# p-mc-grath/DMMFODS

Measured on AMD Instinct MI355X. Metric: training images/sec at 1280x1920 RGB+LiDAR, higher is better.
Workload: dtype f16; 1 GPU; C2 d121 early-fusion 6ch b4 1280x1920; key=c2, per_gpu_batch=4, global_batch=4, height=1280, width=1920, storage_dtype=fp16, accumulate=fp32, parallelism=dp1, weights=random-init (reference init, seed 123)

## Files before the change

dmmfods_amd/csrc/bw1.hip:

```cpp
#include <algorithm>
#include <cstdio>
#include <cstdlib>
#include <type_traits>

#include "common.h"
#include "dispatch.h"
#include "gather.h"
#include "isa.h"
#include "pointwise.h"

namespace dmm {

#ifndef B1_DBG
#define B1_DBG 0
#endif
#ifndef B1_LATE_PREFETCH
#define B1_LATE_PREFETCH 0
#endif
#ifndef B1_RAW_BAR
#define B1_RAW_BAR 0
#endif
#ifndef B1_NT
#define B1_NT 0
#endif
// ... 264 lines not shown
      }
    };
    if (cvalid) { if (UNC && full) finish(std::true_type()); else finish(std::false_type()); }
    fold_to_lds<16, SLOT, B1_CT>(s1, s2, red, cs, cvalid, lane);
    }
#if B1_RAW_BAR
    lds_barrier();
#else
    __syncthreads();
#endif
  }

  if (tid < B1_CT && c0 + tid < a.N) {
    const size_t rep = (size_t)(blockIdx.x & (STAT_REPS - 1)) * a.stat_stride;
    const double S1 = red[fold_slot<16, SLOT>(0, tid)];
    double S2 = red[fold_slot<16, SLOT>(1, tid)];
    if constexpr (UNC) S2 = (S2 - (double)kc[2 * B1_CT + tid] * S1) * (double)kc[3 * B1_CT + tid];
    atomic_add_f64(a.red1 + rep + c0 + tid, S1);
    atomic_add_f64(a.red2 + rep + c0 + tid, S2);
  }
  const int c = c0 + 32 * wave + r;
  if constexpr (PART) {
    float* slot = g.part + ((size_t)split * g.nct + ct) * B1_SLOT_FLOATS + (size_t)wave * (B1_NB * 32);
#pragma unroll
    for (int j = 0; j < 4; ++j)
#pragma unroll
      for (int i = 0; i < 16; ++i) {
        const int n = 32 * j + (i & 3) + 8 * (i >> 2) + 4 * h;
        slot[n * 32 + r] = accw[j][i];
      }
  } else if (!(B1_DBG & 1) && c < g.wC) {
    const size_t chunk = (size_t)(c0 / 32 + wave);
#pragma unroll
    for (int j = 0; j < 4; ++j)
#pragma unroll
      for (int i = 0; i < 16; ++i) {
        const int n = 32 * j + (i & 3) + 8 * (i >> 2) + 4 * h;
        atomic_add_f32(g.dpack + (chunk * g.dNpad + n) * 32 + r, accw[j][i]);
      }
  }
  if (B1_DBG & 1) {
    float s = 0.f;
#pragma unroll
    for (int j = 0; j < 4; ++j)
#pragma unroll
      for (int i = 0; i < 16; ++i) s += accw[j][i];
    if (s == 1.2345e33f) g.dpack[0] = s;
  }
}

template <typename T, int PQ, bool ACC, bool PART>
static hipError_t launch_bw1_t(const Bw1Args& g, int nwg, hipStream_t st) {
  return launch_lds<bw1_kernel<T, PQ, ACC, PART>>(B1_LDS, nwg, NTHREADS, B1_LDS, st, g);
}

bool bw1_eligible(const WgradArgs& w, const ConvArgs& d, int dtype, unsigned deny) {
  if (((deny >> IMPL_BW1) & 1u) || dtype == DT_F32 || w.nseg != 1 || d.nseg != 1 || d.pool2) return false;
  const Seg& wx = w.seg[0];
  const Seg& wg = w.dy;
  const Seg& dg = d.seg[0];
  if (wx.mode != G_PLAIN || wx.istride != 1 || wx.ntaps != 1 || wx.taps[0] != 0 || wx.scale == nullptr || wx.C % 32) return false;
  if (wg.mode != G_PLAIN || wg.istride != 1 || wg.ntaps != 1 || wg.taps[0] != 0 || wg.scale != nullptr || wg.C != B1_NB) return false;
  if (dg.mode != G_PLAIN || dg.istride != 1 || dg.ntaps != 1 || dg.taps[0] != 0 || dg.scale != nullptr || dg.C != B1_NB || dg.Cpad != B1_NB) return false;
  if (dg.src != wg.src || dg.ld != wg.ld || dg.q != wg.q || dg.src2 != wg.src2) return false;
  if (w.N != B1_NB || w.Npad != B1_NB || w.M != d.M || d.N != wx.C || d.Npad % 32) return false;
  if (d.bx != wx.src || d.ldbx != wx.ld || d.bscale != wx.scale || d.bshift != wx.shift) return false;
  if (d.out == nullptr || d.ostride != 1 || d.Hout != d.Ho || d.Wout != d.Wo || wx.Hs != d.Ho || wx.Ws != d.Wo) return false;
  const double span = 2.0 * (double)d.M;
  if (span * d.ldbx >= 4294967296.0 || span * d.ldo >= 4294967296.0 || span * dg.ld >= 4294967296.0 || span * dg.ld2 >= 4294967296.0) return false;
  return true;
}

Bw1Geom bw1_geometry(const ConvArgs& a) {
  Bw1Geom q;
  q.nct = (a.N + B1_CT - 1) / B1_CT;
  q.ntiles = (a.M + B1_TM - 1) / B1_TM;
  constexpr int cus = DESIGN_CUS;
  static const int per_cu = lab_int("DMM_BW1_PER_CU", 2);
  int nsplit = std::max(1, (per_cu * cus + q.nct - 1) / q.nct);
  nsplit = std::min(nsplit, std::max(1, q.ntiles / 4));
  q.tiles_per_wg = (q.ntiles + nsplit - 1) / nsplit;
  q.nsplit = (q.ntiles + q.tiles_per_wg - 1) / q.tiles_per_wg;
  q.xcd_group = (q.nct > 1 && q.nsplit >= 32 && q.tiles_per_wg >= 8) ? 1 : 0;
  q.nwg = q.xcd_group ? ((q.nsplit + 7) / 8) * 8 * q.nct : q.nsplit * q.nct;
  return q;
}

static bool g_bw1_part = !lab_flag("DMM_NO_BW1_PART");

static bool bw1_uses_part(const Bw1Args& g, const Bw1Geom& q) {
  return g_bw1_part && g.part != nullptr && q.nsplit * q.nct <= g.part_slots && q.nsplit > 1;
}

hipError_t launch_bw1(const Bw1Args& g0, int dtype, hipStream_t st) {
  Bw1Args g = g0;
  const ConvArgs& a = g.c;
  if (a.M <= 0) return hipSuccess;
  const Bw1Geom q = bw1_geometry(a);
  note_impl(IMPL_BW1);
  g.nct = q.nct; g.ntiles = q.ntiles; g.tiles_per_wg = q.tiles_per_wg; g.xcd_group = q.xcd_group; g.nsplit = q.nsplit;
  const int nwg = q.nwg;
  const int pq = a.seg[0].q ? 2 : 0;
  const bool acc = a.accumulate != 0;
  const bool part = bw1_uses_part(g, q);
#define B1_GO(T) \
  (part ? (pq ? (acc ? launch_bw1_t<T, 2, true, true>(g, nwg, st) : launch_bw1_t<T, 2, false, true>(g, nwg, st))     \
              : (acc ? launch_bw1_t<T, 0, true, true>(g, nwg, st) : launch_bw1_t<T, 0, false, true>(g, nwg, st)))    \
        : (pq ? (acc ? launch_bw1_t<T, 2, true, false>(g, nwg, st) : launch_bw1_t<T, 2, false, false>(g, nwg, st))   \
              : (acc ? launch_bw1_t<T, 0, true, false>(g, nwg, st) : launch_bw1_t<T, 0, false, false>(g, nwg, st))))
  if (dtype == DT_F16) return B1_GO(f16);
  return B1_GO(bf16);
#undef B1_GO
}

__global__ __launch_bounds__(256) void bw1_reduce_kernel(const float* __restrict__ part, float* __restrict__ dpack, int nct, int nsplit, int nfloats) {
  const int e = (blockIdx.x * 256 + threadIdx.x) * 4;
  if (e >= nct * B1_SLOT_FLOATS) return;
  f32x4 s = {0.f, 0.f, 0.f, 0.f};
  const float* p = part + e;
  const size_t pitch = (size_t)nct * B1_SLOT_FLOATS;
  int k = 0;
  for (; k + 16 <= nsplit; k += 16) {
    f32x4 v[16];
#pragma unroll
    for (int u = 0; u < 16; ++u) v[u] = __builtin_nontemporal_load((const f32x4*)(p + (size_t)(k + u) * pitch));
#pragma unroll
    for (int u = 0; u < 16; u += 4) s += (v[u] + v[u + 1]) + (v[u + 2] + v[u + 3]);
  }
  for (; k + 4 <= nsplit; k += 4) {
    const f32x4 v0 = *(const f32x4*)(p + (size_t)k * pitch), v1 = *(const f32x4*)(p + (size_t)(k + 1) * pitch);
    const f32x4 v2 = *(const f32x4*)(p + (size_t)(k + 2) * pitch), v3 = *(const f32x4*)(p + (size_t)(k + 3) * pitch);
    s += (v0 + v1) + (v2 + v3);
  }
  for (; k < nsplit; ++k) s += *(const f32x4*)(p + (size_t)k * pitch);
  if (e < nfloats) *(f32x4*)(dpack + e) = s;
}

hipError_t launch_bw1_reduce(const Bw1Args& g, hipStream_t st) {
  const ConvArgs& a = g.c;
  if (a.M <= 0) return hipSuccess;
  const Bw1Geom q = bw1_geometry(a);
  if (!bw1_uses_part(g, q)) return hipSuccess;
  const int nfloats = ((g.wC + 31) / 32) * g.dNpad * 32;
  const int nthreads = q.nct * B1_SLOT_FLOATS / 4;
  hipLaunchKernelGGL(bw1_reduce_kernel, dim3((nthreads + 255) / 256), dim3(256), 0, st, g.part, g.dpack, q.nct, q.nsplit, nfloats);
  return hipGetLastError();
}

}
```

dmmfods_amd/csrc/conv3.hip:

```cpp
#include <algorithm>
#include <cstdio>
#include <cstdlib>
#include <type_traits>

#include "common.h"
#include "dispatch.h"
#include "gather.h"
#include "isa.h"

namespace dmm {

constexpr int C3_TH = 8, C3_TW = 16;
#ifndef C3_DBG
#define C3_DBG 0
#endif
constexpr int C3_WRING = 3;
#ifndef C3_RAW_EPI_BAR
#define C3_RAW_EPI_BAR 0
#endif

struct Conv3Args {
  ConvArgs c;
  int tiles_y, tiles_x, ntiles;
  int dymin0, dxmin0;
// ... 271 lines not shown
      for (int gc = 0; gc < GC; ++gc) {
        const int ck = grp * GC + gc;
        if (ck < NCH) {
#pragma unroll
          for (int s = 0; s < 2; ++s) {
            V av = z;
            if constexpr (SEG0) {
              if (ck < NCH0) av = *(const V*)(halo + abase + toffs[ck / (SEG0 ? CG : 1)] + (ck % (SEG0 ? CG : 1)) * 64 + s * 32);
            }
            if constexpr (SEG1) if (ck >= NCH0) {
              const int o = off1[2 * (ck - NCH0) + s];
              const V ld = *(const V*)(halo1 + (o >= 0 ? o : 0));
              av = o >= 0 ? ld : z;
            }
#pragma unroll
            for (int t = 0; t < NT; ++t) {
              const V bv = *(const V*)(Bp + (gc * BN + 32 * t + r) * 64 + (((2 * s + h) ^ bsw) << 4));
              acc[t] = mma16(av, bv, acc[t]);
            }
          }
        }
      }
    }
    if (grp + 2 < NGRP) vm_lds_barrier<NPW>();
    else vm_lds_barrier<0>();
  }
  constexpr bool PERSIST = EPI == EPI_STORE;
  const int lnext = lt + gridDim.x;
  const bool more = PERSIST && lnext < nitems;
  if (more) { decode(lnext); load_halo(); }
  if (!((C3_DBG & 8) && acc[0][0] != 123.f)) {
  T* Cs = (T*)smem;
  constexpr int CPITCH = BN + 8;
  float ps1[NT], ps2[NT];
#pragma unroll
  for (int t = 0; t < NT; ++t) {
    ps1[t] = 0.f; ps2[t] = 0.f;
#pragma unroll
    for (int i = 0; i < 16; ++i) {
      const int row = 32 * wave + (i & 3) + 8 * (i >> 2) + 4 * h;
      const T v = from_f32<T>(acc[t][i]);
      Cs[row * CPITCH + 32 * t + r] = v;
      if (EPI == EPI_STORE && rowpix[row] >= 0) { const float f = to_f32(v); ps1[t] += f; ps2[t] = fmaf(f, f, ps2[t]); }
    }
  }
  if constexpr (EPI == EPI_STORE) {
#pragma unroll
    for (int t = 0; t < NT; ++t) {
      wpart[(wave * 2 + h) * BN + 32 * t + r] = fold_swap32(ps1[t], ps2[t]);
    }
  }
  if constexpr (PERSIST && C3_RAW_EPI_BAR) lds_barrier();
  else __syncthreads();

  if constexpr (EPI == EPI_STORE) {
    T* out = (T*)a.out;
#pragma unroll
    for (int i = 0; i < NIT; ++i) {
      const int row = rr + RPP * i;
      const int pix = rowpix[row];
      if (pix < 0 || !colvalid) continue;
      *(V*)(out + (size_t)pix * a.ldo + n) = *(const V*)(Cs + row * CPITCH + cv * SLOT);
    }
    if (!(a.stat_sum == nullptr || (C3_DBG & 32)))
    if (!(C3_DBG & 16) && tid < 2 * BN) {
      const int col = tid % BN, which = tid / BN;
      if (col < a.N) {
        double s = 0.0;
#pragma unroll
        for (int w = 0; w < 4; ++w) s += (double)wpart[(w * 2 + which) * BN + col];
        red[tid] += s;
      }
    }
  } else {
    float s1[SLOT], s2[SLOT];
#pragma unroll
    for (int i = 0; i < SLOT; ++i) { s1[i] = 0.f; s2[i] = 0.f; }
    T* gout = (T*)a.out;
    float sc[SLOT], sh[SLOT], mu[SLOT], is[SLOT];
    if (colvalid) {
      load_f32s<SLOT>(a.bscale + n, sc); load_f32s<SLOT>(a.bshift + n, sh);
      load_f32s<SLOT>(a.bmean + n, mu); load_f32s<SLOT>(a.binvstd + n, is);
    }
    constexpr bool TWO_PASS = !SEG0 && SEG1;
    const bool fin = TWO_PASS && a.eq != nullptr;
    float qv[TWO_PASS ? SLOT : 1], rv[TWO_PASS ? SLOT : 1];
    if constexpr (TWO_PASS) {
#pragma unroll
      for (int e = 0; e < SLOT; ++e) { qv[e] = 0.f; rv[e] = 0.f; }
      if (fin && colvalid) { load_f32s<SLOT>(a.eq + n, qv); load_f32s<SLOT>(a.er + n, rv); }
    }
#pragma unroll
    for (int i = 0; i < NIT; ++i) {
      if (ppre[i] < 0) continue;
      const int row = rr + RPP * i;
      float av[SLOT], xf[SLOT], gf[SLOT];
      vec_to_f32<T>(*(const V*)(Cs + row * CPITCH + cv * SLOT), av);
      vec_to_f32<T>(xpre[i], xf);
      if (a.accumulate && gout != nullptr) vec_to_f32<T>(*(const V*)(gout + (size_t)ppre[i] * a.ldo + n), gf);
#pragma unroll
      for (int e = 0; e < SLOT; ++e) {
        const float dz = (fmaf(xf[e], sc[e], sh[e]) > 0.f) ? av[e] : 0.f;
        s1[e] += dz;
        s2[e] = fmaf(dz, (xf[e] - mu[e]) * is[e], s2[e]);
        gf[e] = ((a.accumulate && gout != nullptr) ? gf[e] : 0.f) + sc[e] * dz;
        if constexpr (TWO_PASS) gf[e] += fmaf(rv[e], xf[e], qv[e]);
      }
      if (gout != nullptr) *(V*)(gout + (size_t)ppre[i] * a.ldo + n) = f32_to_vec<T>(gf);
    }
    if (a.red1 != nullptr) {
      fold_to_lds<NCV, SLOT, BN>(s1, s2, red, cv, colvalid, lane);
      __syncthreads();
      if (!(C3_DBG & (16 | 32)) && tid < BN && tid < a.N) {
        const size_t rep = (size_t)(blockIdx.x & (STAT_REPS - 1)) * a.stat_stride;
        atomic_add_f64(a.red1 + rep + tid, red[fold_slot<NCV, SLOT>(0, tid)]);
        atomic_add_f64(a.red2 + rep + tid, red[fold_slot<NCV, SLOT>(1, tid)]);
      }
    }
  }
  }
  if (!more) break;
  lt = lnext;
  if constexpr (PERSIST && C3_RAW_EPI_BAR) lds_barrier();
  else __syncthreads();
  }
  if constexpr (EPI == EPI_STORE) {
    if (!(a.stat_sum == nullptr || (C3_DBG & (16 | 32))) && tid < 2 * BN) {
      const int col = tid % BN, which = tid / BN;
      if (col < a.N) {
        const size_t rep = (size_t)(blockIdx.x & (STAT_REPS - 1)) * a.stat_stride;
        atomic_add_f64((which ? a.stat_sq : a.stat_sum) + rep + col, red[tid]);
      }
    }
  }
}

typedef hipError_t (*C3Inst)(const Conv3Args& g, hipStream_t st);

template <typename T, int CS, int SPAN, int TSPAN, int TSTR, int NT, int GC, int EPI, int PRO>
static hipError_t launch_c3(const Conv3Args& g, hipStream_t st) {
  typedef Conv3Cfg<T, CS, SPAN, TSPAN, TSTR, NT, GC> SM;
  static_assert(SM::bytes <= 80 * 1024, "two workgroups per CU");
  constexpr auto kern = conv3_kernel<T, CS, SPAN, TSPAN, TSTR, NT, GC, EPI, PRO>;
  const hipError_t e = lds_limit<kern>(SM::bytes > 48 * 1024 ? SM::bytes : 0);
  if (e != hipSuccess) return e;
  static const int cus = device_cus();
  static const int rounds = lab_int("DMM_C3_ROUNDS", 1);
  const int per_cu = std::min(4, (160 * 1024) / SM::bytes);
  int nwg = g.ntiles * (g.c.nphase > 0 ? g.c.nphase : 1);
  if (EPI == EPI_STORE && rounds > 0 && nwg > per_cu * cus * rounds) nwg = per_cu * cus * rounds / 8 * 8;
  return launch_lds<kern>(0, nwg, NTHREADS, SM::bytes, st, g);
}

template <typename T>
static C3Inst c3_instance(int epi, int pro, int cs, int span, int tspan, int tstr, int nt) {
  if (epi == EPI_STORE && pro == 1) {
    if (tspan < 0 && span == 2 && nt == 1 && cs == 16) return launch_c3<T, 16, 2, -1, 1, 1, 4, EPI_STORE, 1>;
    if (tspan < 0 && span == 2 && nt == 1 && cs == 8) return launch_c3<T, 8, 2, -1, 1, 1, 2, EPI_STORE, 1>;
    if (tspan == 2 && tstr == 2 && span == 1 && nt == 2 && cs == 16) return launch_c3<T, 16, 1, 2, 2, 2, 2, EPI_STORE, 1>;
  }
  if (epi == EPI_BNBWD && tspan < 0 && span == 2) {
    if (cs == 4 && nt == 4 && pro == 2) return launch_c3<T, 4, 2, -1, 1, 4, 1, EPI_BNBWD, 2>;
    if (cs == 4 && nt == 4 && pro == 0) return launch_c3<T, 4, 2, -1, 1, 4, 1, EPI_BNBWD, 0>;
    if (cs == 4 && nt == 2 && pro == 2) return launch_c3<T, 4, 2, -1, 1, 2, 1, EPI_BNBWD, 2>;
    if (cs == 4 && nt == 2 && pro == 0) return launch_c3<T, 4, 2, -1, 1, 2, 1, EPI_BNBWD, 0>;
    if (cs == 8 && nt == 1 && pro == 0) return launch_c3<T, 8, 2, -1, 1, 1, 2, EPI_BNBWD, 0>;
    if (cs == 8 && nt == 1 && pro == 2) return launch_c3<T, 8, 2, -1, 1, 1, 2, EPI_BNBWD, 2>;
  }
  if (epi == EPI_STORE && cs == 0 && tspan == 6 && tstr == 2 && pro == 0 && nt == 2) return launch_c3<T, 0, 0, 6, 2, 2, 2, EPI_STORE, 0>;
  if (epi == EPI_BNBWD && cs == 0 && tspan == 4 && tstr == 1 && pro == 0) {
    if (nt == 2) return launch_c3<T, 0, 0, 4, 1, 2, 2, EPI_BNBWD, 0>;
    if (nt == 1) return launch_c3<T, 0, 0, 4, 1, 1, 2, EPI_BNBWD, 0>;
  }
  return nullptr;
}

static bool tap_box(const Seg& sg, int& dymin, int& dxmin, int& span) {
  int dymax = -128, dxmax = -128;
  dymin = 127; dxmin = 127;
  for (int t = 0; t < sg.ntaps; ++t) {
    const int dy = (int)(signed char)(sg.taps[t] & 0xff), dx = (int)(signed char)((sg.taps[t] >> 8) & 0xff);
    dymin = dy < dymin ? dy : dymin; dymax = dy > dymax ? dy : dymax;
    dxmin = dx < dxmin ? dx : dxmin; dxmax = dx > dxmax ? dx : dxmax;
  }
  span = dymax - dymin;
  if (span < 0 || span > 6 || dxmax - dxmin != span || sg.ntaps != (span + 1) * (span + 1)) return false;
  bool seen[49] = {false};
  for (int t = 0; t < sg.ntaps; ++t) {
    const int dy = (int)(signed char)(sg.taps[t] & 0xff) - dymin, dx = (int)(signed char)((sg.taps[t] >> 8) & 0xff) - dxmin;
    if (seen[dy * (span + 1) + dx]) return false;
    seen[dy * (span + 1) + dx] = true;
  }
  return true;
}

struct Conv3Launch {
  Conv3Args g;
  C3Inst run;
  int shape[8];
};

bool conv3_resolve(const ConvArgs& a, int dtype, int epi, Resolved& r) {
  if (dtype == DT_F32 || a.nseg < 1 || a.nseg > 2 || a.pool2 || (epi != EPI_STORE && epi != EPI_BNBWD)) return false;
  const Seg& sg = a.seg[0];
  if (a.Npad % 32 || a.Npad > 128) return false;
  Conv3Launch& l = r.put<Conv3Launch>();
  Conv3Args& g = l.g;
  g.c = a;
  g.dymin0 = g.dxmin0 = g.dymin1 = g.dxmin1 = 0;
  int cs = 0, span = 0, tspan = -1, tstr = 1;
  auto thin_ok = [&](const Seg& s1, int stride) {
    return s1.mode == G_PLAIN && s1.istride == stride && s1.C == 8 && s1.Cpad == 8 && s1.Hs == stride * a.Ho && s1.Ws == stride * a.Wo &&
           s1.q == nullptr && tap_box(s1, g.dymin1, g.dxmin1, tspan);
  };
  if (a.nseg == 1 && sg.C == 8 && sg.istride == 2) {
    tstr = 2;
    if (epi != EPI_STORE || !thin_ok(sg, 2) || tspan != 6 || sg.scale != nullptr) return false;
  } else if (a.nseg == 1 && sg.C == 8) {
    if (!thin_ok(sg, 1) || tspan != 4 || sg.scale != nullptr) return false;
  } else {
    if (sg.mode != G_PLAIN || sg.istride != 1 || sg.C % 32 || sg.Cpad != sg.C || sg.Hs != a.Ho || sg.Ws != a.Wo) return false;
    if (!tap_box(sg, g.dymin0, g.dxmin0, span) || span < 1 || span > 2) return false;
    cs = sg.C / 8;
    if (a.nseg == 2) {
      tstr = 2;
      if (!thin_ok(a.seg[1], 2) || tspan != 2 || (a.seg[1].scale != nullptr) != (sg.scale != nullptr)) return false;
    }
  }
  if (a.nphase < 0 || a.nphase > 4) return false;
  if (a.nphase > 0) {
    if (epi != EPI_STORE || a.nseg != 2 || sg.ntaps != 4 || a.seg[1].ntaps != 9) return false;
    for (int ph = 0; ph < a.nphase; ++ph) {
      Seg t0 = sg, t1 = a.seg[1];
      for (int t = 0; t < 4; ++t) t0.taps[t] = a.ph_taps0[ph][t];
      for (int t = 0; t < 9; ++t) t1.taps[t] = a.ph_taps1[ph][t];
      int y0, x0, y1, x1, sp0, sp1;
      if (!tap_box(t0, y0, x0, sp0) || sp0 != span || !tap_box(t1, y1, x1, sp1) || sp1 != tspan || a.ph_wpack[ph] == nullptr ||
          a.ph_py[ph] < 0 || a.ph_py[ph] >= a.ostride || a.ph_px[ph] < 0 || a.ph_px[ph] >= a.ostride)
        return false;
      g.ph_dymin0[ph] = (signed char)y0; g.ph_dxmin0[ph] = (signed char)x0; g.ph_dymin1[ph] = (signed char)y1; g.ph_dxmin1[ph] = (signed char)x1;
    }
  }
  if (a.nseg == 1 && (a.ostride != 1 || a.Hout != a.Ho || a.Wout != a.Wo)) return false;
  if (cs == 0 && tspan == 6 && a.Npad != 64) return false;
  const int pro = sg.scale ? 1 : (sg.q ? 2 : 0);
  if (epi == EPI_BNBWD && a.accumulate && a.out == nullptr) return false;
  if ((a.eq != nullptr) != (a.er != nullptr)) return false;
  if (a.eq != nullptr && !(epi == EPI_BNBWD && cs == 0 && tspan == 4 && tstr == 1 && pro == 0 && a.out != nullptr && !a.accumulate &&
                           a.red1 == nullptr && a.red2 == nullptr))
    return false;
  g.tiles_y = (a.Ho + C3_TH - 1) / C3_TH;
  g.tiles_x = (a.Wo + C3_TW - 1) / C3_TW;
  g.ntiles = a.B * g.tiles_y * g.tiles_x;
  const int nt = a.Npad / 32;
  const int shape[8] = {epi, pro, cs, span, tspan, tstr, nt, a.M};
// ... 16 lines not shown
```

dmmfods_amd/csrc/pointwise.hip:

```cpp
#include <type_traits>

#include "common.h"
#include "gather.h"
#include "pointwise.h"

namespace dmm {

thread_local int g_last_impl = IMPL_AUTO;
thread_local unsigned g_impl_mask = 0;

template <typename T>
__global__ __launch_bounds__(256) void convert_input_kernel(ConvertArgs a) {
  __shared__ double red[16];
  if (threadIdx.x < 16) red[threadIdx.x] = 0.0;
  __syncthreads();
  const size_t plane = (size_t)a.H * a.W;
  const size_t npix = (size_t)a.B * plane;
  double s1[8], s2[8];
#pragma unroll
  for (int c = 0; c < 8; ++c) { s1[c] = 0.0; s2[c] = 0.0; }
  const float scale = a.dyn_scale != nullptr ? a.scale * *a.dyn_scale : a.scale;
  for (size_t p = (size_t)blockIdx.x * blockDim.x + threadIdx.x; p < npix; p += (size_t)gridDim.x * blockDim.x) {
    const size_t b = p / plane, rem = p - b * plane;
    float v[8];
// ... 98 lines not shown
      int b, oy, ox;
      row_to_byx(p, a.Hp, a.Wp, b, oy, ox);
      float best[SLOT];
      int arg[SLOT];
#pragma unroll
      for (int i = 0; i < SLOT; ++i) { best[i] = -INFINITY; arg[i] = 0; }
      V win[9];
      bool ok[9];
#pragma unroll
      for (int k = 0; k < 9; ++k) {
        const int iy = 2 * oy - 1 + k / 3, ix = 2 * ox - 1 + k % 3;
        ok[k] = iy >= 0 && ix >= 0 && iy < a.H0 && ix < a.W0;
        const int cy = ok[k] ? iy : 2 * oy, cx = ok[k] ? ix : 2 * ox;
        win[k] = *(const V*)(y0 + ((size_t)(b * a.H0 + cy) * a.W0 + cx) * a.ld0 + c);
      }
#pragma unroll
      for (int k = 0; k < 9; ++k) {
        float f[SLOT];
        vec_to_f32<T>(win[k], f);
#pragma unroll
        for (int i = 0; i < SLOT; ++i) {
          const float v = fmaxf(fmaf(f[i], sc[i], sh[i]), 0.f);
          if (ok[k] && v > best[i]) { best[i] = v; arg[i] = k; }
        }
      }
      const V ov = f32_to_vec<T>(best);
      *(V*)(out + (size_t)p * a.ldo + c) = ov;
      float r[SLOT];
      vec_to_f32<T>(ov, r);
      unsigned long long packed = 0;
#pragma unroll
      for (int i = 0; i < SLOT; ++i) {
        packed |= (unsigned long long)(unsigned)arg[i] << (8 * i);
        s1[i] += (double)r[i];
        s2[i] += (double)r[i] * (double)r[i];
      }
      if constexpr (SLOT == 8) *(unsigned long long*)(a.argmax + (size_t)p * a.C + c) = packed;
      else *(unsigned*)(a.argmax + (size_t)p * a.C + c) = (unsigned)packed;
    }
  }
  block_channel_reduce<SLOT>(red, a.C, c, s1, s2, a.stat_sum, a.stat_sq, a.stat_stride);
}

hipError_t launch_maxpool_fwd(const MaxpoolArgs& a, int dtype, hipStream_t st) {
  const int slot = dtype == DT_F32 ? 4 : 8;
  const int rpb = 256 / (a.C / slot);
  const int npix = a.B * a.Hp * a.Wp;
  int grid = (npix + rpb - 1) / rpb;
  if (grid > 2048) grid = 2048;
  const size_t smem = 2 * a.C * sizeof(double);
  if (dtype == DT_F16) hipLaunchKernelGGL(maxpool_fwd_kernel<f16>, dim3(grid), dim3(256), smem, st, a);
  else if (dtype == DT_BF16) hipLaunchKernelGGL(maxpool_fwd_kernel<bf16>, dim3(grid), dim3(256), smem, st, a);
  else hipLaunchKernelGGL(maxpool_fwd_kernel<float>, dim3(grid), dim3(256), smem, st, a);
  return hipGetLastError();
}

template <typename T>
__global__ __launch_bounds__(256) void maxpool_bwd_kernel(MaxpoolBwdArgs a) {
  constexpr int SLOT = TT<T>::SLOT;
  typedef typename TT<T>::vec V;
  extern __shared__ double red[];
  for (int i = threadIdx.x; i < 2 * a.C; i += blockDim.x) red[i] = 0.0;
  __syncthreads();
  const int ncv = a.C / SLOT;
  const int cv = threadIdx.x % ncv, rl = threadIdx.x / ncv, rpb = blockDim.x / ncv;
  const int c = cv * SLOT;
  float sc[SLOT], sh[SLOT], q[SLOT], rr[SLOT], qlo[SLOT], rlo[SLOT];
  double s1[SLOT], s2[SLOT];
  load_f32s<SLOT>(a.scale + c, sc);
  load_f32s<SLOT>(a.shift + c, sh);
  load_f32s<SLOT>(a.q + c, q);
  load_f32s<SLOT>(a.r + c, rr);
  load_f32s<SLOT>(a.ql + c, qlo);
  load_f32s<SLOT>(a.rl + c, rlo);
  float mu[SLOT], istd[SLOT];
  load_f32s<SLOT>(a.mean + c, mu);
  load_f32s<SLOT>(a.invstd + c, istd);
#pragma unroll
  for (int i = 0; i < SLOT; ++i) { s1[i] = 0.0; s2[i] = 0.0; }
  float f1[SLOT], f2[SLOT];
#pragma unroll
  for (int i = 0; i < SLOT; ++i) { f1[i] = 0.f; f2[i] = 0.f; }
  int pending = 0;
  const int npix = a.B * a.H0 * a.W0;
  const T* y0 = (const T*)a.y0;
  const T* gp = (const T*)a.gpool;
  const T* xp = (const T*)a.xpool;
  T* gy0 = (T*)a.gy0;
  if (rl < rpb) {
    const int stride = gridDim.x * rpb;
    int sb, sy, sx;
    row_to_byx(stride, a.H0, a.W0, sb, sy, sx);
    int b, y, x;
    row_to_byx(blockIdx.x * rpb + rl, a.H0, a.W0, b, y, x);
    for (int p = blockIdx.x * rpb + rl; p < npix; p += stride) {
      float g[SLOT];
#pragma unroll
      for (int i = 0; i < SLOT; ++i) g[i] = 0.f;
      const int oy0 = y >> 1, oy1 = (y + 1) >> 1;
      const int ox0 = x >> 1, ox1 = (x + 1) >> 1;
      V wg[4], wx_[4];
      unsigned long long wam[4];
      bool wok[4];
      int wk[4];
#pragma unroll
      for (int w = 0; w < 4; ++w) {
        const int wy = (w >> 1) ? oy1 : oy0, wx = (w & 1) ? ox1 : ox0;
        wok[w] = ((w >> 1) == 0 || oy1 != oy0) && ((w & 1) == 0 || ox1 != ox0) && wy < a.Hp && wx < a.Wp;
        const int cy = min(wy, a.Hp - 1), cx = min(wx, a.Wp - 1);
        wk[w] = (y - (2 * wy - 1)) * 3 + (x - (2 * wx - 1));
        const size_t op = (size_t)(b * a.Hp + cy) * a.Wp + cx;
        wg[w] = *(const V*)(gp + op * a.ldg + c);
        wx_[w] = *(const V*)(xp + op * a.ldg + c);
        if constexpr (SLOT == 8) wam[w] = *(const unsigned long long*)(a.argmax + op * a.C + c);
        else wam[w] = *(const unsigned*)(a.argmax + op * a.C + c);
      }
      const V y0v = *(const V*)(y0 + (size_t)p * a.ld0 + c);
#pragma unroll
      for (int w = 0; w < 4; ++w) {
        if constexpr (std::is_same<T, f16>::value) {
          typedef unsigned u32x4 __attribute__((ext_vector_type(4)));
          const u32x4 gi = __builtin_bit_cast(u32x4, wg[w]), xi = __builtin_bit_cast(u32x4, wx_[w]);
          const float one = 1.f;
#pragma unroll
          for (int pr = 0; pr < 4; ++pr) {
            float t0, t1, v0, v1;
            asm("v_fma_mix_f32 %0, %1, %2, %3 op_sel_hi:[1,0,0]" : "=v"(t0) : "v"(xi[pr]), "v"(rr[2 * pr]), "v"(q[2 * pr]));
            asm("v_fma_mix_f32 %0, %1, %2, %3 op_sel:[1,0,0] op_sel_hi:[1,0,0]" : "=v"(t1) : "v"(xi[pr]), "v"(rr[2 * pr + 1]), "v"(q[2 * pr + 1]));
            asm("v_fma_mix_f32 %0, %1, %2, %3 op_sel_hi:[1,0,0]" : "=v"(v0) : "v"(gi[pr]), "v"(one), "v"(t0));
            asm("v_fma_mix_f32 %0, %1, %2, %3 op_sel:[1,0,0] op_sel_hi:[1,0,0]" : "=v"(v1) : "v"(gi[pr]), "v"(one), "v"(t1));
            if (wok[w] && (int)((wam[w] >> (16 * pr)) & 0xff) == wk[w]) g[2 * pr] += v0;
            if (wok[w] && (int)((wam[w] >> (16 * pr + 8)) & 0xff) == wk[w]) g[2 * pr + 1] += v1;
          }
        } else {
        float gf[SLOT], xf[SLOT];
        vec_to_f32<T>(wg[w], gf);
        vec_to_f32<T>(wx_[w], xf);
#pragma unroll
        for (int i = 0; i < SLOT; ++i)
          if (wok[w] && (int)((wam[w] >> (8 * i)) & 0xff) == wk[w]) g[i] += (gf[i] + fmaf(rr[i], xf[i], q[i])) + fmaf(rlo[i], xf[i], qlo[i]);
        }
      }
      float yf[SLOT], o[SLOT];
      vec_to_f32<T>(y0v, yf);
#pragma unroll
      for (int i = 0; i < SLOT; ++i) {
        const float dz = (fmaf(yf[i], sc[i], sh[i]) > 0.f) ? g[i] : 0.f;
        f1[i] += dz;
        f2[i] = fmaf(dz, (yf[i] - mu[i]) * istd[i], f2[i]);
        o[i] = sc[i] * dz;
      }
      *(V*)(gy0 + (size_t)p * a.ld0 + c) = f32_to_vec<T>(o);
      if (++pending == 8) {
        pending = 0;
#pragma unroll
        for (int i = 0; i < SLOT; ++i) { s1[i] += (double)f1[i]; s2[i] += (double)f2[i]; f1[i] = 0.f; f2[i] = 0.f; }
      }
      x += sx; if (x >= a.W0) { x -= a.W0; ++y; }
      y += sy; if (y >= a.H0) { y -= a.H0; ++b; }
      b += sb;
    }
#pragma unroll
    for (int i = 0; i < SLOT; ++i) { s1[i] += (double)f1[i]; s2[i] += (double)f2[i]; }
  }
  block_channel_reduce<SLOT>(red, a.C, c, s1, s2, a.red1, a.red2, a.stat_stride);
}

hipError_t launch_maxpool_bwd(const MaxpoolBwdArgs& a, int dtype, hipStream_t st) {
  const int slot = dtype == DT_F32 ? 4 : 8;
  const int rpb = 256 / (a.C / slot);
  const int npix = a.B * a.H0 * a.W0;
  int grid = (npix + rpb - 1) / rpb;
  static const int cap = lab_int("DMM_MPB_GRID", 2048);
  if (grid > cap) grid = cap;
  const size_t smem = 2 * a.C * sizeof(double);
  if (dtype == DT_F16) hipLaunchKernelGGL(maxpool_bwd_kernel<f16>, dim3(grid), dim3(256), smem, st, a);
  else if (dtype == DT_BF16) hipLaunchKernelGGL(maxpool_bwd_kernel<bf16>, dim3(grid), dim3(256), smem, st, a);
  else hipLaunchKernelGGL(maxpool_bwd_kernel<float>, dim3(grid), dim3(256), smem, st, a);
  return hipGetLastError();
}

__device__ __forceinline__ void loss_elem(const BceArgs& a, int n, float x, float t, float& loss, float& dx) {
  float bce, dbce;
  if (!a.from_prob) {
    const float e = expf(-fabsf(x));
    bce = fmaxf(x, 0.f) - x * t + log1pf(e);
    const float sig = x >= 0.f ? 1.f / (1.f + e) : e / (1.f + e);
    dbce = sig - t;
  } else {
    const float lp = fmaxf(logf(x), -100.f), lq = fmaxf(log1pf(-x), -100.f);
    bce = -(t * lp + (1.f - t) * lq);
    dbce = (x - t) / fmaxf((1.f - x) * x, 1e-12f);
  }
  if (a.kind == 0) { loss = bce; dx = dbce; return; }
  const float al = a.alpha[n], ga = a.gamma[n];
  const float omp = fmaxf(-expm1f(-bce), 0.f);
  const float pt = 1.f - omp;
  const float pw = powf(omp, ga);
  const float ratio = omp > 0.f ? bce / omp : 1.f;
  loss = al * pw * bce;
  dx = al * pw * dbce * fmaf(ga * pt, ratio, 1.f);
}

template <typename T>
__global__ __launch_bounds__(256) void bce_metrics_kernel(BceArgs a) {
  __shared__ float red[4 * 8];
  if (threadIdx.x < 32) red[threadIdx.x] = 0.f;
  __syncthreads();
  const int b = blockIdx.y;
  const size_t plane = (size_t)a.H * a.W;
  float ls[8], eq[8], in_[8], un[8];
#pragma unroll
  for (int n = 0; n < 8; ++n) { ls[n] = eq[n] = in_[n] = un[n] = 0.f; }
  const bool vec4 = (plane & 3) == 0 && ((((uintptr_t)a.logits) | ((uintptr_t)a.target)) & 15) == 0 && a.loss_out == nullptr && a.dx_out == nullptr;
  const size_t nthreads = (size_t)gridDim.x * blockDim.x, gid = (size_t)blockIdx.x * blockDim.x + threadIdx.x;
  const float gscale = a.dyn_scale != nullptr ? a.loss_scale * *a.dyn_scale : a.loss_scale;
  if (vec4) {
    for (size_t p = gid * 4; p < plane; p += nthreads * 4) {
      f32x4 xv[8], tv[8];
#pragma unroll
      for (int n = 0; n < 8; ++n)
        if (n < a.NC) {
          const size_t idx = ((size_t)b * a.NC + n) * plane + p;
          xv[n] = *(const f32x4*)(a.logits + idx);
          tv[n] = *(const f32x4*)(a.target + idx);
        }
      float g[4][8];
#pragma unroll
      for (int n = 0; n < 8; ++n) {
#pragma unroll
        for (int j = 0; j < 4; ++j) g[j][n] = 0.f;
        if (n < a.NC) {
#pragma unroll
          for (int j = 0; j < 4; ++j) {
            const float x = xv[n][j], t = tv[n][j];
            float l, d;
            loss_elem(a, n, x, t, l, d);
            ls[n] += l;
            g[j][n] = d * gscale;
            const bool pp = x >= a.thr, gg = t >= a.thr;
            eq[n] += (pp == gg) ? 1.f : 0.f;
            in_[n] += (pp && gg) ? 1.f : 0.f;
            un[n] += (pp || gg) ? 1.f : 0.f;
          }
        }
      }
      if (a.dlogits != nullptr) {
        T* d = (T*)a.dlogits + ((size_t)b * plane + p) * 8;
#pragma unroll
        for (int j = 0; j < 4; ++j)
#pragma unroll
          for (int n = 0; n < 8; ++n) d[j * 8 + n] = from_f32<T>(g[j][n]);
      }
    }
  } else
// ... 377 lines not shown
```

Before: 161.0 img/s.

## Add 5x5 walk kernel for BN-backward conv, restructure maxpool backward per pooled block

Three independent changes. First, the bw1 geometry now raises tiles-per-workgroup until the grid fits per_cu*CUs slots. Second, a new persistent 5x5 conv kernel with LDS-resident weights and a single halo stage replaces the generic tspan=4 BN-backward conv3 path, and the two-pass correction term moves into it (removed from conv3's generic epilogue). Third, maxpool backward iterates over pooled output blocks and scatters to a 2x2 input quad instead of gathering 4 windows per input pixel, cutting redundant window loads at the cost of more register pressure.

```diff
diff --git a/dmmfods_amd/csrc/bw1.hip b/dmmfods_amd/csrc/bw1.hip
--- a/dmmfods_amd/csrc/bw1.hip
+++ b/dmmfods_amd/csrc/bw1.hip
@@ -370,6 +370,10 @@
   q.tiles_per_wg = (q.ntiles + nsplit - 1) / nsplit;
   q.nsplit = (q.ntiles + q.tiles_per_wg - 1) / q.tiles_per_wg;
   q.xcd_group = (q.nct > 1 && q.nsplit >= 32 && q.tiles_per_wg >= 8) ? 1 : 0;
+  while (q.nsplit * q.nct > per_cu * cus && q.nsplit > 1) {
+    ++q.tiles_per_wg;
+    q.nsplit = (q.ntiles + q.tiles_per_wg - 1) / q.tiles_per_wg;
+  }
   q.nwg = q.xcd_group ? ((q.nsplit + 7) / 8) * 8 * q.nct : q.nsplit * q.nct;
   return q;
 }
diff --git a/dmmfods_amd/csrc/conv3.hip b/dmmfods_amd/csrc/conv3.hip
--- a/dmmfods_amd/csrc/conv3.hip
+++ b/dmmfods_amd/csrc/conv3.hip
@@ -377,14 +377,6 @@
       load_f32s<SLOT>(a.bscale + n, sc); load_f32s<SLOT>(a.bshift + n, sh);
       load_f32s<SLOT>(a.bmean + n, mu); load_f32s<SLOT>(a.binvstd + n, is);
     }
-    constexpr bool TWO_PASS = !SEG0 && SEG1;
-    const bool fin = TWO_PASS && a.eq != nullptr;
-    float qv[TWO_PASS ? SLOT : 1], rv[TWO_PASS ? SLOT : 1];
-    if constexpr (TWO_PASS) {
-#pragma unroll
-      for (int e = 0; e < SLOT; ++e) { qv[e] = 0.f; rv[e] = 0.f; }
-      if (fin && colvalid) { load_f32s<SLOT>(a.eq + n, qv); load_f32s<SLOT>(a.er + n, rv); }
-    }
 #pragma unroll
     for (int i = 0; i < NIT; ++i) {
       if (ppre[i] < 0) continue;
@@ -399,7 +391,6 @@
         s1[e] += dz;
         s2[e] = fmaf(dz, (xf[e] - mu[e]) * is[e], s2[e]);
         gf[e] = ((a.accumulate && gout != nullptr) ? gf[e] : 0.f) + sc[e] * dz;
-        if constexpr (TWO_PASS) gf[e] += fmaf(rv[e], xf[e], qv[e]);
       }
       if (gout != nullptr) *(V*)(gout + (size_t)ppre[i] * a.ldo + n) = f32_to_vec<T>(gf);
     }
@@ -426,6 +417,212 @@
         const size_t rep = (size_t)(blockIdx.x & (STAT_REPS - 1)) * a.stat_stride;
         atomic_add_f64((which ? a.stat_sq : a.stat_sum) + rep + col, red[tid]);
       }
+    }
+  }
+}
+
+template <int NT>
+struct Conv5Cfg {
+  static constexpr int BN = 32 * NT, NCH = 7, NTAPS = 25;
+  static constexpr int HH1 = C3_TH + 4, HW1 = C3_TW + 4, NSL1 = HH1 * HW1;
+  static constexpr int RP1 = HW1 * 16;
+  static constexpr int W = NCH * BN * 64;
+  static constexpr int HALO = NSL1 * 16;
+  static constexpr int STAGE = BM * (BN + 8) * 2;
+  static constexpr int RED = 2 * BN * 8;
+  static constexpr int KC = 6 * BN * 4;
+  static constexpr int bytes = W + HALO + STAGE + RED + KC;
+  static_assert(NSL1 <= NTHREADS, "one halo slot per thread");
+};
+
+template <typename T, int NT>
+__global__ __launch_bounds__(NTHREADS, 3) void conv5d_walk_kernel(const Conv3Args g) {
+  typedef typename TT<T>::vec V;
+  typedef Conv5Cfg<NT> SM;
+  constexpr int SLOT = 8, BN = SM::BN, NCH = SM::NCH, NT1 = SM::NTAPS, RP1 = SM::RP1;
+  constexpr int NP = NCH * BN / 16;
+  constexpr int NCV = BN / SLOT;
+  constexpr int RPP = NTHREADS / NCV;
+  constexpr int NIT = BM / RPP;
+  constexpr int CPITCH = BN + 8;
+  const ConvArgs& a = g.c;
+  const Seg& sg1 = a.seg[0];
+
+  extern __shared__ __attribute__((aligned(16))) unsigned char smem[];
+  unsigned char* wres = smem;
+  unsigned char* halo1 = smem + SM::W;
+  T* Cs = (T*)(smem + SM::W + SM::HALO);
+  double* red = (double*)(smem + SM::W + SM::HALO + SM::STAGE);
+  float* kc = (float*)(smem + SM::W + SM::HALO + SM::STAGE + SM::RED);
+
+  const int tid = threadIdx.x, lane = tid & 63, wave = tid >> 6;
+  const int r = lane & 31, h = lane >> 5;
+
+  {
+    const T* wp = (const T*)a.wpack;
+    const unsigned lds0 = (unsigned)(size_t)(__attribute__((address_space(3))) unsigned char*)smem;
+#pragma unroll
+    for (int q = 0; q < (NP + 3) / 4; ++q) {
+      const int p = __builtin_amdgcn_readfirstlane(wave + 4 * q);
+      if (p < NP) lds_dma16(wp + (16 * p + (lane >> 2)) * 32 + (((lane & 3) ^ ((lane >> 4) & 3)) << 3),
+                          __builtin_amdgcn_readfirstlane(lds0 + p * 1024));
+    }
+  }
+  if (tid < BN) {
+    const bool v = tid < a.N;
+    kc[tid] = v ? a.bscale[tid] : 0.f; kc[BN + tid] = v ? a.bshift[tid] : 0.f;
+    kc[2 * BN + tid] = v ? a.bmean[tid] : 0.f; kc[3 * BN + tid] = v ? a.binvstd[tid] : 0.f;
+    kc[4 * BN + tid] = (v && a.eq != nullptr) ? a.eq[tid] : 0.f; kc[5 * BN + tid] = (v && a.eq != nullptr) ? a.er[tid] : 0.f;
+  }
+  if (tid < 2 * BN) red[tid] = 0.0;
+
+  int lt = blockIdx.x;
+  int b, y0, x0;
+  auto decode = [&](int l) {
+    int tile = xcd_remap(l, g.ntiles);
+    const int tx_i = tile % g.tiles_x; tile /= g.tiles_x;
+    const int ty_i = tile % g.tiles_y;
+    b = tile / g.tiles_y;
+    y0 = ty_i * C3_TH; x0 = tx_i * C3_TW;
+  };
+  const int cv = tid % NCV, rr = tid / NCV;
+  const int n = cv * SLOT;
+  const bool colvalid = n < a.N;
+  const int hy = tid / SM::HW1, hx = tid - hy * SM::HW1;
+  V z;
+#pragma unroll
+  for (int e = 0; e < SLOT; ++e) z[e] = (T)0;
+  auto request = [&](V& hv, bool& hk, int (&pp)[NIT], V (&xv)[NIT]) {
+    const int sy = y0 + g.dymin1 + hy, sx = x0 + g.dxmin1 + hx;
+    hk = tid < SM::NSL1 && (unsigned)sy < (unsigned)sg1.Hs && (unsigned)sx < (unsigned)sg1.Ws;
+    const int cy = min(max(sy, 0), sg1.Hs - 1), cx = min(max(sx, 0), sg1.Ws - 1);
+    hv = *(const V*)((const T*)sg1.src + ((size_t)(b * sg1.Hs + cy) * sg1.Ws + cx) * sg1.ld);
+    const T* bx = (const T*)a.bx;
+#pragma unroll
+    for (int i = 0; i < NIT; ++i) {
+      const int row = rr + RPP * i;
+      const int y = y0 + row / C3_TW, x = x0 + row % C3_TW;
+      pp[i] = (colvalid && y < a.Ho && x < a.Wo) ? (b * a.Hout + y * a.ostride + a.py) * a.Wout + x * a.ostride + a.px : -1;
+      xv[i] = z;
+      if (pp[i] >= 0) xv[i] = *(const V*)(bx + (size_t)pp[i] * a.ldbx + n);
+    }
+  };
+  V hraw, xpre[NIT], xnext[NIT];
+  bool hok;
+  int ppre[NIT], pnext[NIT];
+  decode(lt);
+  request(hraw, hok, ppre, xpre);
+
+  const int ty = 2 * wave + (r >> 4), tx = r & 15;
+  const int bsw = (r >> 2) & 3;
+  const int abase1 = (ty - g.dymin1) * RP1 + (tx - g.dxmin1) * 16;
+  int toff[2 * NCH][2];
+#pragma unroll
+  for (int c = 0; c < NCH; ++c)
+#pragma unroll
+    for (int s = 0; s < 2; ++s)
+#pragma unroll
+      for (int hh = 0; hh < 2; ++hh) {
+        const int j = 4 * c + 2 * s + hh;
+        const int t = sg1.taps[j < NT1 ? j : 0];
+        toff[2 * c + s][hh] = (int)(signed char)(t & 0xff) * RP1 + (int)(signed char)((t >> 8) & 0xff) * 16;
+      }
+  T* gout = (T*)a.out;
+  __builtin_amdgcn_s_waitcnt(0x0f70);
+
+  while (true) {
+    if (tid < SM::NSL1) *(V*)(halo1 + tid * 16) = hok ? hraw : z;
+    lds_barrier();
+
+    f32x16 acc[NT];
+#pragma unroll
+    for (int t = 0; t < NT; ++t)
+#pragma unroll
+      for (int i = 0; i < 16; ++i) acc[t][i] = 0.f;
+#pragma unroll
+    for (int ck = 0; ck < NCH; ++ck)
+#pragma unroll
+      for (int s = 0; s < 2; ++s) {
+        const int j0 = 4 * ck + 2 * s;
+        V av = z;
+        if (j0 < NT1) {
+          const V ld = *(const V*)(halo1 + abase1 + (h ? toff[2 * ck + s][1] : toff[2 * ck + s][0]));
+          av = (j0 + h < NT1) ? ld : z;
+        }
+#pragma unroll
+        for (int t = 0; t < NT; ++t) {
+          const V bv = *(const V*)(wres + (ck * BN + 32 * t + r) * 64 + (((2 * s + h) ^ bsw) << 4));
+          acc[t] = mma16(av, bv, acc[t]);
+        }
+      }
+
+    const int lnext = lt + gridDim.x;
+    const bool more = lnext < g.ntiles;
+    if (more) { decode(lnext); request(hraw, hok, pnext, xnext); }
+
+#pragma unroll
+    for (int t = 0; t < NT; ++t)
+#pragma unroll
+      for (int i = 0; i < 16; ++i) {
+        const int row = 32 * wave + (i & 3) + 8 * (i >> 2) + 4 * h;
+        Cs[row * CPITCH + 32 * t + r] = from_f32<T>(acc[t][i]);
+      }
+    lds_barrier();
+
+    float s1[SLOT], s2[SLOT];
+#pragma unroll
+    for (int i = 0; i < SLOT; ++i) { s1[i] = 0.f; s2[i] = 0.f; }
+    typedef T T4 __attribute__((ext_vector_type(4)));
+    V ov[NIT];
+#pragma unroll
+    for (int i = 0; i < NIT; ++i) ov[i] = z;
+#pragma unroll
+    for (int hf = 0; hf < 2; ++hf) {
+      float sc[4], sh[4], mu[4], is[4], qv[4], rv[4];
+      load_f32s<4>(kc + n + 4 * hf, sc); load_f32s<4>(kc + BN + n + 4 * hf, sh);
+      load_f32s<4>(kc + 2 * BN + n + 4 * hf, mu); load_f32s<4>(kc + 3 * BN + n + 4 * hf, is);
+      load_f32s<4>(kc + 4 * BN + n + 4 * hf, qv); load_f32s<4>(kc + 5 * BN + n + 4 * hf, rv);
+#pragma unroll
+      for (int i = 0; i < NIT; ++i) {
+        if (ppre[i] < 0) continue;
+        const int row = rr + RPP * i;
+        const T4 a4 = *(const T4*)(Cs + row * CPITCH + cv * SLOT + 4 * hf);
+        V gold = z;
+        if (a.accumulate && gout != nullptr) gold = *(const V*)(gout + (size_t)ppre[i] * a.ldo + n);
+#pragma unroll
+        for (int e = 0; e < 4; ++e) {
+          const int ch = 4 * hf + e;
+          const float av = to_f32(a4[e]), xf = to_f32(xpre[i][ch]);
+          const float dz = (fmaf(xf, sc[e], sh[e]) > 0.f) ? av : 0.f;
+          s1[ch] += dz;
+          s2[ch] = fmaf(dz, (xf - mu[e]) * is[e], s2[ch]);
+          float gf = ((a.accumulate && gout != nullptr) ? to_f32(gold[ch]) : 0.f) + sc[e] * dz;
+          gf += fmaf(rv[e], xf, qv[e]);
+          ov[i][ch] = from_f32<T>(gf);
+        }
+      }
+    }
+    if (a.red1 != nullptr) fold_to_lds<NCV, SLOT, BN>(s1, s2, red, cv, colvalid, lane);
+    if (more) {
+#pragma unroll
+      for (int i = 0; i < NIT; ++i) xpre[i] = xnext[i];
+    }
+    if (gout != nullptr) {
+#pragma unroll
+      for (int i = 0; i < NIT; ++i)
+        if (ppre[i] >= 0) *(V*)(gout + (size_t)ppre[i] * a.ldo + n) = ov[i];
+    }
+    if (!more) break;
+    lt = lnext;
+#pragma unroll
+    for (int i = 0; i < NIT; ++i) ppre[i] = pnext[i];
+  }
+  if (a.red1 != nullptr) {
+    __syncthreads();
+    if (tid < BN && tid < a.N) {
+      const size_t rep = (size_t)(blockIdx.x & (STAT_REPS - 1)) * a.stat_stride;
+      atomic_add_f64(a.red1 + rep + tid, red[fold_slot<NCV, SLOT>(0, tid)]);
+      atomic_add_f64(a.red2 + rep + tid, red[fold_slot<NCV, SLOT>(1, tid)]);
     }
   }
 }
@@ -447,6 +644,19 @@
   return launch_lds<kern>(0, nwg, NTHREADS, SM::bytes, st, g);
 }
 
+template <typename T, int NT>
+static hipError_t launch_c5walk(const Conv3Args& g, hipStream_t st) {
+  typedef Conv5Cfg<NT> SM;
+  static_assert(SM::bytes <= 54 * 1024, "three workgroups per CU");
+  constexpr auto kern = conv5d_walk_kernel<T, NT>;
+  const hipError_t e = lds_limit<kern>(SM::bytes > 48 * 1024 ? SM::bytes : 0);
+  if (e != hipSuccess) return e;
+  static const int cus = device_cus();
+  static const int per_cu = lab_int("DMM_C5_PER_CU", 3);
+  const int cap = std::max(8, per_cu * cus / 8 * 8);
+  return launch_lds<kern>(0, std::min(g.ntiles, cap), NTHREADS, SM::bytes, st, g);
+}
+
 template <typename T>
 static C3Inst c3_instance(int epi, int pro, int cs, int span, int tspan, int tstr, int nt) {
   if (epi == EPI_STORE && pro == 1) {
@@ -464,8 +674,8 @@
   }
   if (epi == EPI_STORE && cs == 0 && tspan == 6 && tstr == 2 && pro == 0 && nt == 2) return launch_c3<T, 0, 0, 6, 2, 2, 2, EPI_STORE, 0>;
   if (epi == EPI_BNBWD && cs == 0 && tspan == 4 && tstr == 1 && pro == 0) {
-    if (nt == 2) return launch_c3<T, 0, 0, 4, 1, 2, 2, EPI_BNBWD, 0>;
-    if (nt == 1) return launch_c3<T, 0, 0, 4, 1, 1, 2, EPI_BNBWD, 0>;
+    if (nt == 2) return launch_c5walk<T, 2>;
+    if (nt == 1) return launch_c5walk<T, 1>;
   }
   return nullptr;
 }
diff --git a/dmmfods_amd/csrc/pointwise.hip b/dmmfods_amd/csrc/pointwise.hip
--- a/dmmfods_amd/csrc/pointwise.hip
+++ b/dmmfods_amd/csrc/pointwise.hip
@@ -204,82 +204,107 @@
 #pragma unroll
   for (int i = 0; i < SLOT; ++i) { f1[i] = 0.f; f2[i] = 0.f; }
   int pending = 0;
-  const int npix = a.B * a.H0 * a.W0;
   const T* y0 = (const T*)a.y0;
   const T* gp = (const T*)a.gpool;
   const T* xp = (const T*)a.xpool;
   T* gy0 = (T*)a.gy0;
+  const int nblk = a.B * a.Hp * a.Wp;
   if (rl < rpb) {
     const int stride = gridDim.x * rpb;
     int sb, sy, sx;
-    row_to_byx(stride, a.H0, a.W0, sb, sy, sx);
-    int b, y, x;
-    row_to_byx(blockIdx.x * rpb + rl, a.H0, a.W0, b, y, x);
-    for (int p = blockIdx.x * rpb + rl; p < npix; p += stride) {
-      float g[SLOT];
-#pragma unroll
-      for (int i = 0; i < SLOT; ++i) g[i] = 0.f;
-      const int oy0 = y >> 1, oy1 = (y + 1) >> 1;
-      const int ox0 = x >> 1, ox1 = (x + 1) >> 1;
+    row_to_byx(stride, a.Hp, a.Wp, sb, sy, sx);
+    int b, k, j;
+    row_to_byx(blockIdx.x * rpb + rl, a.Hp, a.Wp, b, k, j);
+    for (int p = blockIdx.x * rpb + rl; p < nblk; p += stride) {
+      const bool wdn = k + 1 < a.Hp, wrt = j + 1 < a.Wp;
       V wg[4], wx_[4];
       unsigned long long wam[4];
-      bool wok[4];
-      int wk[4];
 #pragma unroll
       for (int w = 0; w < 4; ++w) {
-        const int wy = (w >> 1) ? oy1 : oy0, wx = (w & 1) ? ox1 : ox0;
-        wok[w] = ((w >> 1) == 0 || oy1 != oy0) && ((w & 1) == 0 || ox1 != ox0) && wy < a.Hp && wx < a.Wp;
-        const int cy = min(wy, a.Hp - 1), cx = min(wx, a.Wp - 1);
-        wk[w] = (y - (2 * wy - 1)) * 3 + (x - (2 * wx - 1));
-        const size_t op = (size_t)(b * a.Hp + cy) * a.Wp + cx;
+        const int wy = ((w >> 1) && wdn) ? k + 1 : k, wx = ((w & 1) && wrt) ? j + 1 : j;
+        const size_t op = (size_t)(b * a.Hp + wy) * a.Wp + wx;
         wg[w] = *(const V*)(gp + op * a.ldg + c);
         wx_[w] = *(const V*)(xp + op * a.ldg + c);
         if constexpr (SLOT == 8) wam[w] = *(const unsigned long long*)(a.argmax + op * a.C + c);
         else wam[w] = *(const unsigned*)(a.argmax + op * a.C + c);
       }
-      const V y0v = *(const V*)(y0 + (size_t)p * a.ld0 + c);
+      const bool pdn = 2 * k + 1 < a.H0, prt = 2 * j + 1 < a.W0;
+      V y0v[4];
+      size_t pix[4];
+#pragma unroll
+      for (int d = 0; d < 4; ++d) {
+        const int y = 2 * k + (((d >> 1) && pdn) ? 1 : 0), x = 2 * j + (((d & 1) && prt) ? 1 : 0);
+        pix[d] = (size_t)(b * a.H0 + y) * a.W0 + x;
+        y0v[d] = *(const V*)(y0 + pix[d] * a.ld0 + c);
+      }
+      float g[4][SLOT];
+#pragma unroll
+      for (int d = 0; d < 4; ++d)
+#pragma unroll
+        for (int i = 0; i < SLOT; ++i) g[d][i] = 0.f;
 #pragma unroll
       for (int w = 0; w < 4; ++w) {
+        const bool wok = ((w >> 1) == 0 || wdn) && ((w & 1) == 0 || wrt);
+        float e[SLOT];
         if constexpr (std::is_same<T, f16>::value) {
           typedef unsigned u32x4 __attribute__((ext_vector_type(4)));
           const u32x4 gi = __builtin_bit_cast(u32x4, wg[w]), xi = __builtin_bit_cast(u32x4, wx_[w]);
           const float one = 1.f;
 #pragma unroll
           for (int pr = 0; pr < 4; ++pr) {
-            float t0, t1, v0, v1;
+            float t0, t1;
             asm("v_fma_mix_f32 %0, %1, %2, %3 op_sel_hi:[1,0,0]" : "=v"(t0) : "v"(xi[pr]), "v"(rr[2 * pr]), "v"(q[2 * pr]));
             asm("v_fma_mix_f32 %0, %1, %2, %3 op_sel:[1,0,0] op_sel_hi:[1,0,0]" : "=v"(t1) : "v"(xi[pr]), "v"(rr[2 * pr + 1]), "v"(q[2 * pr + 1]));
-            asm("v_fma_mix_f32 %0, %1, %2, %3 op_sel_hi:[1,0,0]" : "=v"(v0) : "v"(gi[pr]), "v"(one), "v"(t0));
-            asm("v_fma_mix_f32 %0, %1, %2, %3 op_sel:[1,0,0] op_sel_hi:[1,0,0]" : "=v"(v1) : "v"(gi[pr]), "v"(one), "v"(t1));
-            if (wok[w] && (int)((wam[w] >> (16 * pr)) & 0xff) == wk[w]) g[2 * pr] += v0;
-            if (wok[w] && (int)((wam[w] >> (16 * pr + 8)) & 0xff) == wk[w]) g[2 * pr + 1] += v1;
+            asm("v_fma_mix_f32 %0, %1, %2, %3 op_sel_hi:[1,0,0]" : "=v"(e[2 * pr]) : "v"(gi[pr]), "v"(one), "v"(t0));
+            asm("v_fma_mix_f32 %0, %1, %2, %3 op_sel:[1,0,0] op_sel_hi:[1,0,0]" : "=v"(e[2 * pr + 1]) : "v"(gi[pr]), "v"(one), "v"(t1));
           }
         } else {
-        float gf[SLOT], xf[SLOT];
-        vec_to_f32<T>(wg[w], gf);
-        vec_to_f32<T>(wx_[w], xf);
-#pragma unroll
-        for (int i = 0; i < SLOT; ++i)
-          if (wok[w] && (int)((wam[w] >> (8 * i)) & 0xff) == wk[w]) g[i] += (gf[i] + fmaf(rr[i], xf[i], q[i])) + fmaf(rlo[i], xf[i], qlo[i]);
+          float gf[SLOT], xf[SLOT];
+          vec_to_f32<T>(wg[w], gf);
+          vec_to_f32<T>(wx_[w], xf);
+#pragma unroll
+          for (int i = 0; i < SLOT; ++i) e[i] = (gf[i] + fmaf(rr[i], xf[i], q[i])) + fmaf(rlo[i], xf[i], qlo[i]);
         }
-      }
-      float yf[SLOT], o[SLOT];
-      vec_to_f32<T>(y0v, yf);
-#pragma unroll
-      for (int i = 0; i < SLOT; ++i) {
-        const float dz = (fmaf(yf[i], sc[i], sh[i]) > 0.f) ? g[i] : 0.f;
-        f1[i] += dz;
-        f2[i] = fmaf(dz, (yf[i] - mu[i]) * istd[i], f2[i]);
-        o[i] = sc[i] * dz;
-      }
-      *(V*)(gy0 + (size_t)p * a.ld0 + c) = f32_to_vec<T>(o);
-      if (++pending == 8) {
+#pragma unroll
+        for (int i = 0; i < SLOT; ++i) {
+          const int am = wok ? (int)((wam[w] >> (8 * i)) & 0xff) : -1;
+          if (w == 0) {
+            if (am == 4) g[0][i] += e[i];
+            if (am == 5) g[1][i] += e[i];
+            if (am == 7) g[2][i] += e[i];
+            if (am == 8) g[3][i] += e[i];
+          } else if (w == 1) {
+            if (am == 3) g[1][i] += e[i];
+            if (am == 6) g[3][i] += e[i];
+          } else if (w == 2) {
+            if (am == 1) g[2][i] += e[i];
+            if (am == 2) g[3][i] += e[i];
+          } else {
+            if (am == 0) g[3][i] += e[i];
+          }
+        }
+      }
+#pragma unroll
+      for (int d = 0; d < 4; ++d) {
+        const bool pok = ((d >> 1) == 0 || pdn) && ((d & 1) == 0 || prt);
+        float yf[SLOT], o[SLOT];
+        vec_to_f32<T>(y0v[d], yf);
+#pragma unroll
+        for (int i = 0; i < SLOT; ++i) {
+          const float dz = (pok && fmaf(yf[i], sc[i], sh[i]) > 0.f) ? g[d][i] : 0.f;
+          f1[i] += dz;
+          f2[i] = fmaf(dz, (yf[i] - mu[i]) * istd[i], f2[i]);
+          o[i] = sc[i] * dz;
+        }
+        if (pok) *(V*)(gy0 + pix[d] * a.ld0 + c) = f32_to_vec<T>(o);
+      }
+      if (++pending == 2) {
         pending = 0;
 #pragma unroll
         for (int i = 0; i < SLOT; ++i) { s1[i] += (double)f1[i]; s2[i] += (double)f2[i]; f1[i] = 0.f; f2[i] = 0.f; }
       }
-      x += sx; if (x >= a.W0) { x -= a.W0; ++y; }
-      y += sy; if (y >= a.H0) { y -= a.H0; ++b; }
+      j += sx; if (j >= a.Wp) { j -= a.Wp; ++k; }
+      k += sy; if (k >= a.Hp) { k -= a.Hp; ++b; }
       b += sb;
     }
 #pragma unroll
@@ -291,8 +316,8 @@
 hipError_t launch_maxpool_bwd(const MaxpoolBwdArgs& a, int dtype, hipStream_t st) {
   const int slot = dtype == DT_F32 ? 4 : 8;
   const int rpb = 256 / (a.C / slot);
-  const int npix = a.B * a.H0 * a.W0;
-  int grid = (npix + rpb - 1) / rpb;
+  const int nblk = a.B * a.Hp * a.Wp;
+  int grid = (nblk + rpb - 1) / rpb;
   static const int cap = lab_int("DMM_MPB_GRID", 2048);
   if (grid > cap) grid = cap;
   const size_t smem = 2 * a.C * sizeof(double);
```

Result: no change. 162.5 img/s (median of 6 runs) (+0.9%).
